# sm-edwards/CrossScale-ECG-A-Modular-HPC-Pipeline-from-Locality-Optimization-to-MPI-GPU-Overlap

Hardware: AMD Instinct MI355X
Metric: ECG samples/sec (node) + conv1d speedup vs torch.Conv1d, tiny 1D-CNN at 1/2/4/8 GPU (higher is better)
Workload: dtype bf16; 1 GPU; model=TinyECG (1458 params), global_batch=256, seq_len=500, parallelism=dp1, sync=fedavg every 50 local steps (none all_reduce AVG, overlap=none), per_client_batch=256, max_windows_per_client=20000, backend=fused

## Files before the change

### crossscale-ecg-a-modular-hpc-pipeline-from-locality-optimization-to-mpi-gpu-overlap_amd/ops/_lib.py

```python
from __future__ import annotations

import ctypes as C
import os
import threading
from typing import Optional

import torch

LIB_DIR = os.environ.get("ECG_LIB_DIR") or os.path.join(os.path.dirname(os.path.dirname(os.path.abspath(__file__))), "_lib")

_lock = threading.Lock()
_libs = {}

vp, i32, i64, f32 = C.c_void_p, C.c_int, C.c_long, C.c_float
u64 = C.c_uint64
f64p = C.POINTER(C.c_double)
i32p = C.POINTER(C.c_int)
i64p = C.POINTER(C.c_int64)

STATUS = {0: "ok", 1: "bad argument", 2: "problem too large for the fused kernel", 3: "HIP runtime error",
          4: "I/O error", 5: "timeout", 6: "end of data"}


class NativeError(RuntimeError):
# ... 9 lines not shown
    with _lock:
        if name in _libs:
            return _libs[name]
        path = os.path.join(LIB_DIR, name)
        lib = None
        if os.path.exists(path):
            lib = C.CDLL(path, mode=C.RTLD_GLOBAL)
        _libs[name] = lib
        return lib


def _sig(lib, name, argtypes, restype=i32):
    fn = getattr(lib, name)
    fn.argtypes = argtypes
    fn.restype = restype
    return fn


class TinyRound(C.Structure):
    _fields_ = [("X", vp), ("ldx", i64), ("idx", vp), ("Y", vp), ("params", vp), ("mom", vp), ("slab", vp),
                ("loss_acc", vp), ("wprep", vp), ("xg", vp), ("yg", vp),
                ("L", i32), ("nc", i32), ("slab_stride", i32), ("B", i32), ("steps", i32),
                ("lr", f32), ("momentum", f32), ("wd", f32), ("nesterov", i32), ("prec", i32),
                ("dp_clip", f32), ("dp_sigma", f32), ("dp_seed", u64), ("dp_scale", vp), ("dp_step", vp)]


def _bind_kernels(lib: C.CDLL) -> None:
    _sig(lib, "ecg_tiny_param_count", [i32])
    _sig(lib, "ecg_tiny_smem_bytes", [i32, i32])
    _sig(lib, "ecg_tiny_step_grads", [vp, i32, i64, vp, vp, vp, i32, vp, i32, i32, f32, i32, vp, vp])
    _sig(lib, "ecg_tiny_forward", [vp, i32, i64, vp, vp, i32, vp, i32, i32, vp, vp])
    _sig(lib, "ecg_tiny_wprep_bytes", [])
    _sig(lib, "ecg_tiny_prep", [vp, vp, vp])
    _sig(lib, "ecg_tiny_eval", [vp, i32, i64, vp, vp, i32, vp, i32, vp, vp, vp, vp, vp, i32, vp])
    _sig(lib, "ecg_tiny_eval_scratch_bytes", [i32])
    _sig(lib, "ecg_tiny_eval_out_bytes", [i32])
    _sig(lib, "ecg_slab_reduce_sgd", [vp, i32, i32, i32, vp, vp, vp, vp, f32, f32, f32, i32, i32, vp, vp])
    _sig(lib, "ecg_slab_reduce_dp_sgd", [vp, i32, i32, i32, vp, vp, vp, vp, f32, f32, f32, i32, i32, vp,
                                         f32, f32, u64, vp, vp, vp])
    _sig(lib, "ecg_dp_noise", [vp, i32, u64, u64, vp])
    native = _sig(lib, "ecg_tiny_round_sizeof", [])()
    if native != C.sizeof(TinyRound):
        raise NativeError(f"EcgTinyRound is {native} bytes in libecg_kernels.so but {C.sizeof(TinyRound)} in "
                          "ops/_lib.py: rebuild the library (python csrc/build.py) or update TinyRound")
    _sig(lib, "ecg_tiny_round_enqueue", [C.POINTER(TinyRound), vp])
    _sig(lib, "ecg_tiny_round_capture", [C.POINTER(vp), C.POINTER(TinyRound)])
    _sig(lib, "ecg_tiny_gather_floats", [i32, i32], i64)
    _sig(lib, "ecg_tiny_step_grads_twice", [vp, i32, i64, vp, vp, vp, i32, vp, i32, i32, f32, i32, vp, vp])
    _sig(lib, "ecg_tiny_force_waves", [i32])
    _sig(lib, "ecg_tiny_set_stamps", [vp])
    _sig(lib, "ecg_round_graph_launch", [vp, vp])
    _sig(lib, "ecg_round_graph_destroy", [vp])
    _sig(lib, "ecg_round_graph_upload", [vp, vp])
    _sig(lib, "conv1d_batch_hip", [vp, vp, vp, i32, i32, i32, vp])
    _sig(lib, "conv1d_batch_hip_sync", [vp, vp, vp, i32, i32, i32, vp])
    _sig(lib, "conv1d_batch_hip_spin", [vp, vp, vp, i32, i32, i32, vp])
    _sig(lib, "conv1d_batch_hip_flag", [vp, vp, vp, i32, i32, i32, vp])
    _sig(lib, "conv1d_valid_dgrad_hip", [vp, vp, vp, i32, i32, i32, vp])
    _sig(lib, "conv1d_valid_dgrad_hip_bf16", [vp, vp, vp, i32, i32, i32, vp])
    _sig(lib, "conv1d_valid_wgrad_ws_floats", [i32, i32, i32], i64)
    _sig(lib, "conv1d_valid_wgrad_hip", [vp, vp, vp, vp, i64, i32, i32, i32, vp])
    _sig(lib, "conv1d_valid_wgrad_hip_bf16", [vp, vp, vp, vp, i64, i32, i32, i32, vp])
    _sig(lib, "conv1d_batch_hip_bf16", [vp, vp, vp, i32, i32, i32, vp])
    _sig(lib, "ecg_sgd_flat", [vp, vp, vp, i64, f32, f32, f32, f32, i32, i32, f32, vp, vp])
    _sig(lib, "ecg_gather_rows_f32", [vp, i64, i32, vp, i32, vp, i64, i32, f32, vp])
    _sig(lib, "ecg_gather_rows_bf16", [vp, i64, i32, vp, i32, vp, i64, i32, f32, vp])
    for extra in ("_bind_conv_mc",):
        fn = globals().get(extra)
        if fn:
            fn(lib)
# ... 91 lines not shown
```

### crossscale-ecg-a-modular-hpc-pipeline-from-locality-optimization-to-mpi-gpu-overlap_amd/ops/fused_tiny.py

```python
from __future__ import annotations

import ctypes as C
import os
from typing import Optional

import torch

from . import _lib
from ..models.tiny_ecg import TinyECG, num_params
from ..data.dataset import DeviceIndexSampler
from ..utils.philox import mix64
from .tiny_eval import EvalResult, TinyEvaluator, evaluate_torch, tiny_evaluate


PRECISION = {"bf16": 0, "fp32": 1}


def prec_id(precision: str) -> int:
    if precision not in PRECISION:
        raise ValueError(f"precision must be one of {list(PRECISION)}, got {precision!r}")
    return PRECISION[precision]


def new_wprep(device) -> torch.Tensor:
# ... 94 lines not shown
    z = torch.empty(P, dtype=torch.float32, device=device)
    st = _lib.kernels().ecg_dp_noise(z.data_ptr(), P, int(seed) & (2 ** 64 - 1), int(t) & (2 ** 64 - 1),
                                     _lib.stream_ptr(z.device))
    _lib.check(st, "ecg_dp_noise")
    return z


def reduce_slab(slab: torch.Tensor, num_classes: int = 2):
    P = num_params(num_classes)
    grad = torch.empty(P, dtype=torch.float32, device=slab.device)
    loss = torch.zeros(1, dtype=torch.float32, device=slab.device)
    lib = _lib.kernels()
    st = lib.ecg_slab_reduce_sgd(slab.data_ptr(), slab.shape[0], slab.shape[1], P, None, None, grad.data_ptr(),
                                 loss.data_ptr(), 0.0, 0.0, 0.0, 0, 0, None, _lib.stream_ptr(slab.device))
    _lib.check(st, "ecg_slab_reduce_sgd")
    return grad, loss


class FusedTinyTrainer:

    def __init__(self, model: TinyECG, x_gpu: torch.Tensor, y_gpu: torch.Tensor, batch_size: int,
                 steps_per_round: int, lr: float = 1e-2, momentum: float = 0.9, weight_decay: float = 0.0,
                 nesterov: bool = False, seed: Optional[int] = None, use_graph: Optional[bool] = None,
                 precision: str = "bf16", prefrag: bool = True, gather: bool = True,
                 dp_clip: float = 0.0, dp_noise: float = 0.0, dp_seed: Optional[int] = None):
        self.device = x_gpu.device
        self.precision = precision
        self.prec = prec_id(precision)
        self.model = model
        self.nc = model.num_classes
        self.params = model.flat if model.flat is not None else model.flatten_parameters()
        if self.params.device != self.device:
            raise ValueError("model and dataset must be on the same device")
        self.P = num_params(self.nc)
        self.x = x_gpu.contiguous()
        self.y32 = labels_int32(y_gpu, self.nc)
        _check_dataset(self.x, self.y32, self.nc)
        self.B = int(batch_size)
        self.S = int(steps_per_round)
        self.lr, self.momentum, self.wd, self.nesterov = float(lr), float(momentum), float(weight_decay), bool(nesterov)
        self.stride = slab_stride(self.nc)
        self.mom = torch.zeros_like(self.params)
        self.slab = torch.empty((self.B, self.stride), dtype=torch.float32, device=self.device)
        self.loss_acc = torch.zeros(1, dtype=torch.float32, device=self.device)
        self.idx_table = torch.zeros((self.S, self.B), dtype=torch.int32, device=self.device)
        self.idx_stage = torch.zeros((self.S, self.B), dtype=torch.int32, device=self.device)
        self._staged: Optional[int] = None
        self._loss_steps = 0
        self.sampler = DeviceIndexSampler(self.x.shape[0], self.B, self.device, seed=seed)
        self.use_graph = (os.environ.get("ECG_TINY_GRAPH", "1") != "0") if use_graph is None else bool(use_graph)
        self._graphs = {}
        self.steps_done = 0
        self._evaluator: Optional[TinyEvaluator] = None
        lib = _lib.kernels()
        L = self.x.shape[1]
        smem = lib.ecg_tiny_smem_bytes(L, self.prec)
        if smem > 160 * 1024:
            raise ValueError(f"window length {L} too long for the fused kernel ({smem} B LDS)")
        self.prefrag = bool(prefrag) and precision == "bf16"
        self.wprep = new_wprep(self.device) if self.prefrag else None
        self.gather = bool(gather) and self.prefrag
        self.xg = self.yg = None
        if self.gather:
            self.xg = torch.zeros(lib.ecg_tiny_gather_floats(L, self.B), dtype=torch.float32, device=self.device)
            self.yg = torch.zeros(2 * self.B, dtype=torch.int32, device=self.device)
        check_dp_args(dp_clip, dp_noise)
        self.dp_clip, self.dp_noise = float(dp_clip), float(dp_noise)
        self.dp = self.dp_clip > 0.0
        self.dp_seed = (mix64(0 if seed is None else seed) if dp_seed is None else int(dp_seed)) & (2 ** 64 - 1)
        self.dp_steps = 0
        self.dp_scale = self.dp_step = None
        if self.dp:
            self.dp_scale = torch.zeros(self.B, dtype=torch.float32, device=self.device)
            self.dp_step = torch.zeros(1, dtype=torch.int64, device=self.device)
        self._round = _lib.TinyRound(
            X=self.x.data_ptr(), ldx=self.x.stride(0), Y=self.y32.data_ptr(), params=self.params.data_ptr(),
            mom=self.mom.data_ptr(), slab=self.slab.data_ptr(), loss_acc=self.loss_acc.data_ptr(),
            wprep=_lib.ptr(self.wprep), xg=_lib.ptr(self.xg), yg=_lib.ptr(self.yg), L=L, nc=self.nc,
            slab_stride=self.stride, B=self.B, lr=self.lr, momentum=self.momentum, wd=self.wd,
            nesterov=int(self.nesterov), prec=self.prec, dp_clip=self.dp_clip, dp_sigma=self.dp_noise,
            dp_seed=self.dp_seed, dp_scale=_lib.ptr(self.dp_scale), dp_step=_lib.ptr(self.dp_step))

    def _round_of(self, n: int, table: torch.Tensor):
        r = self._round
        r.idx, r.steps = table.data_ptr(), n
        return C.byref(r)

    def _graph_for(self, n: int, table: torch.Tensor) -> C.c_void_p:
        key = (n, table.data_ptr())
        g = self._graphs.get(key)
        if g is None:
            g = C.c_void_p()
            torch.cuda.synchronize(self.device)
            _lib.check(_lib.kernels().ecg_tiny_round_capture(C.byref(g), self._round_of(n, table)),
                       "ecg_tiny_round_capture")
            self._graphs[key] = g
        return g

    def close(self):
        graphs, self._graphs = getattr(self, "_graphs", {}), {}
        for g in graphs.values():
            if g.value:
                _lib.kernels().ecg_round_graph_destroy(g)

# ... 100 lines not shown
```

### csrc/kernels/tiny_ecg_step.hip

```cpp
#include "../include/ecg_common.h"
#include "../include/tiny_ecg.h"

#include <climits>
#include <cstdint>
#include <cstdlib>
#include <cstring>
#include <type_traits>

namespace {

using namespace ecg::tiny;

constexpr int MAX_PAIRS_PER_WAVE = 4;

struct Smem {
  int Lp;
  int xs_off, xcol_off, h1_off, dh2_off, ps_off, frag_off, red_off, bytes;
};

constexpr int RED_G = 0;
constexpr int RED_POOLED = 16;
constexpr int RED_POOL = 48;

struct FusedOpt {
  int slab_wt;
};
__host__ __device__ constexpr int msplit(int waves) { return (waves - 1) / 5 < 1 ? 1 : (waves - 1) / 5; }
__host__ __device__ constexpr int red_cnt(int waves) { return RED_POOL + waves * 16; }
__host__ __device__ constexpr int red_m(int waves) { return red_cnt(waves) + waves * 16; }
__host__ __device__ constexpr int red_dw1(int waves) { return red_m(waves) + msplit(waves) * 1280; }
__host__ __device__ constexpr int red_head(int waves) { return red_dw1(waves) + waves * 128; }
__host__ __device__ constexpr int red_floats(int waves) { return red_head(waves) + 288; }

__device__ __forceinline__ void st_wt(__amdgpu_buffer_rsrc_t r, int idx, float v) {
  __builtin_amdgcn_raw_buffer_store_b32(__builtin_bit_cast(unsigned, v), r, idx * 4, 0, 16);
}
__device__ __forceinline__ void st_wt4(__amdgpu_buffer_rsrc_t r, int idx, f32x4 v) {
  typedef int i32x4 __attribute__((ext_vector_type(4)));
  __builtin_amdgcn_raw_buffer_store_b128(__builtin_bit_cast(i32x4, v), r, idx * 4, 0, 16);
}
__device__ __forceinline__ float ld_wt(__amdgpu_buffer_rsrc_t r, int idx) {
  return __builtin_bit_cast(float, __builtin_amdgcn_raw_buffer_load_b32(r, idx * 4, 0, 16));
}
constexpr int kOobByte = 0x40000000;

constexpr int F32_KSTEPS = C * K2 / 4;

__host__ __device__ constexpr bool frag_pad_is_bias(int which, int l, int j) { return which == 0 && j == 0 && l < 48; }

__device__ __forceinline__ void wprep_put(unsigned char* wp, int i, float v) {
  __bf16* wb = reinterpret_cast<__bf16*>(wp);
  if (i < C * K1) {
    wb[WP_AW1 + (i / K1) * 8 + i % K1] = ecg::to_bf16(v);
  } else if (i < C * K1 + C) {
    wb[WP_AW1 + (i - C * K1) * 8 + 7] = ecg::to_bf16(v);
  } else if (i < kParamsW2End) {
    const int e = i - (C * K1 + C);
    const int co = e / (C * K2), ci = (e / K2) % C, k = e % K2;
    const int rf = 16 * k + ci, rd = 16 * k + co;
    const __bf16 bv = ecg::to_bf16(v);
    wb[WP_FRAGF + ((rf >> 5) * 64 + 16 * ((rf & 31) >> 3) + co) * 8 + (rf & 7)] = bv;
    wb[WP_FRAGD + ((rd >> 5) * 64 + 16 * ((rd & 31) >> 3) + ci) * 8 + (rd & 7)] = bv;
  } else if (i < kParamsW2End + C) {
    reinterpret_cast<float*>(wp + WP_B2_BYTE)[i - kParamsW2End] = v;
    wb[WP_FRAGF + frag_bias_elem(i - kParamsW2End)] = ecg::to_bf16(v);
  }
}
// ... 17 lines not shown
  s.h1_off = s.xcol_off + (f32 ? 0 : (s.Lp + 1) * 16);
  const int act_bytes = (s.Lp + 8) * C * (f32 ? 4 : 2);
  s.dh2_off = s.h1_off + act_bytes;
  s.ps_off = s.dh2_off + act_bytes;
  const int ps_bytes = ((make_layout(nc).P) * 4 + 15) / 16 * 16;
  s.frag_off = s.ps_off + ps_bytes;
  s.red_off = s.frag_off + (f32 ? 2 * F32_KSTEPS * 64 * 4 : 2 * 3 * 64 * 16);
  s.bytes = s.red_off + (red_floats(waves) * 4 + 15) / 16 * 16;
  return s;
}

__device__ __forceinline__ bf16x8 cat44(s16x4 a, s16x4 b) {
  typedef short s16x8 __attribute__((ext_vector_type(8)));
  s16x8 r;
  r[0] = a[0]; r[1] = a[1]; r[2] = a[2]; r[3] = a[3];
  r[4] = b[0]; r[5] = b[1]; r[6] = b[2]; r[7] = b[3];
  return __builtin_bit_cast(bf16x8, r);
}

__device__ __forceinline__ s16x4 lds_tr16(const __bf16* p) {
  return __builtin_amdgcn_ds_read_tr16_b64_v4i16((__attribute__((address_space(3))) s16x4*)(p));
}

template <int WAVES, bool F32, bool PF = false>
struct TinySample {
  static_assert(!(PF && F32), "prepared fragments are bf16 operands");
  using AT = std::conditional_t<F32, float, __bf16>;
  static constexpr int NT = WAVES * 64;
  Smem sm;
  Layout lay;
  int L, Lp, NP, nc;
  int tid, lane, w, h, c;
  float* xs;
  __bf16* xcol;
  AT* h1s;
  AT* ms;
  float* ps;
  __bf16* fragF;
  __bf16* fragD;
  float* fragF32;
  float* fragD32;
  float* red;
  uint32_t mask1 = 0u;
  bf16x8 pf_aw, pf_wf[3], pf_wd[3];

  __device__ __forceinline__ void load_aw(const float* __restrict__ params) {
#pragma unroll
    for (int j = 0; j < 8; ++j) {
      const float v = j < K1 ? params[lay.w1 + c * K1 + j] : params[lay.b1 + c];
// ... 48 lines not shown
  __device__ __forceinline__ void load_x(const float* __restrict__ xrow, XRegs& r) const {
#pragma unroll
    for (int k = 0; k < XK; ++k) {
      const int i = tid + k * NT, t = i - 3;
      if (k * NT < Lp + 16) {
        const float v = xrow[min(max(t, 0), L - 1)];
        r.v[k] = (i < Lp + 16 && t >= 0 && t < L) ? v : 0.f;
      }
    }
  }
  __device__ __forceinline__ void put_x(const XRegs& r) {
#pragma unroll
    for (int k = 0; k < XK; ++k) {
      const int i = tid + k * NT;
      if (i < Lp + 16) xs[i] = r.v[k];
    }
  }
  __device__ __forceinline__ void stage_x(const float* __restrict__ xrow) {
    XRegs r;
    load_x(xrow, r);
    put_x(r);
  }

  struct X1 {
    float v[2][K1];
  };
  __device__ __forceinline__ int conv1_t(int pi, int u) const {
    return 16 * min(w + (pi + u) * WAVES, Lp / 16 - 1) + (lane & 15);
  }
  __device__ __forceinline__ void conv1_load(__amdgpu_buffer_rsrc_t xr, int pi, X1& r) const {
#pragma unroll
    for (int u = 0; u < 2; ++u) {
      const int t = conv1_t(pi, u);
      const int base = (h == 0 && t < L) ? 4 * max(t - 3, 0) : kOobByte;
#pragma unroll
      for (int j = 0; j < K1; ++j) r.v[u][j] = ld_bounded(xr, base + 4 * j);
    }
  }
  __device__ __forceinline__ bf16x8 conv1_operand(const float (&ld)[K1], int t) const {
    float v[K1];
#pragma unroll
    for (int j = 0; j < K1; ++j) v[j] = ld[j];
    if (h == 0 && t < 3) {
      const int s = 3 - t;
#pragma unroll
      for (int j = K1 - 1; j >= 0; --j) v[j] = (s & 1) ? (j >= 1 ? v[j - 1] : 0.f) : v[j];
#pragma unroll
      for (int j = K1 - 1; j >= 0; --j) v[j] = (s & 2) ? (j >= 2 ? v[j - 2] : 0.f) : v[j];
    }
    bf16x8 Bx;
#pragma unroll
    for (int j = 0; j < K1; ++j) Bx[j] = ecg::to_bf16(v[j]);
    Bx[7] = ecg::to_bf16(h == 0 && t < L ? 1.f : 0.f);
    return Bx;
  }

  __device__ __forceinline__ void put_param(int i, float v) {
    ps[i] = v;
    if constexpr (!F32) {
      if (i >= lay.b2 && i < lay.b2 + C) fragF[frag_bias_elem(i - lay.b2)] = ecg::to_bf16(v);
// ... 20 lines not shown
        if (!frag_pad_is_bias(which, l, j)) (which ? fragD : fragF)[(2 * 64 + l) * 8 + j] = ecg::to_bf16(0.f);
      }
      if (tid < 4) reinterpret_cast<uint32_t*>(xcol + Lp * 8)[tid] = 0u;
    }
    constexpr int DW = C * (int)sizeof(AT) / 4;
    uint32_t* h1w = reinterpret_cast<uint32_t*>(h1s);
    uint32_t* mw = reinterpret_cast<uint32_t*>(ms);
    for (int i = tid; i < 8 * DW; i += NT) {
      const int r = i / DW, d = i % DW;
      const int hr = r < 2 ? r : Lp + 2 + (r - 2);
      h1w[hr * DW + d] = 0u;
      const int dr = r < 4 ? r : Lp + 4 + (r - 4);
      mw[dr * DW + d] = 0u;
    }
  }

  __device__ __forceinline__ void conv1_pair(int pi, const X1& x) {
    const bool has2 = w + (pi + 1) * WAVES < Lp / 16;
    bf16x8 Bx[2];
    int t[2];
#pragma unroll
    for (int u = 0; u < 2; ++u) {
      t[u] = conv1_t(pi, u);
      Bx[u] = conv1_operand(x.v[u], t[u]);
      if (h == 0) *reinterpret_cast<bf16x8*>(xcol + t[u] * 8) = Bx[u];
    }
#pragma unroll
    for (int u = 0; u < 2; ++u) {
      if (u == 1 && !has2) break;
      const f32x4 acc = __builtin_amdgcn_mfma_f32_16x16x32_bf16(pf_aw, Bx[u], f32x4{0.f, 0.f, 0.f, 0.f}, 0, 0, 0);
      bf16x4 o;
#pragma unroll
      for (int i = 0; i < 4; ++i) o[i] = (AT)fmaxf(acc[i], 0.f);
      *reinterpret_cast<bf16x4*>(h1s + (t[u] + 2) * C + 4 * h) = o;
    }
  }
  __device__ __forceinline__ void conv1_mfma(__amdgpu_buffer_rsrc_t xr, const X1& x0) {
    const int ntiles = Lp / 16;
    if (w < ntiles) conv1_pair(0, x0);
#pragma unroll 1
    for (int pi = 2; pi < 2 * MAX_PAIRS_PER_WAVE; pi += 2) {
      if (w + pi * WAVES >= ntiles) break;
      X1 x;
      conv1_load(xr, pi, x);
      conv1_pair(pi, x);
    }
  }
// ... 412 lines not shown

  __device__ __forceinline__ void row_store(__amdgpu_buffer_rsrc_t r, int rowbase) const {
    constexpr int NQ = C * C * K2 / 4;
    static_assert(NQ + 128 + C <= NT || WAVES < 16, "one job per thread at 16 waves");
    if (tid < NQ) {
      const int e0 = 4 * tid;
      f32x4 v = *reinterpret_cast<const f32x4*>(red + red_m(WAVES) + e0);
#pragma unroll
      for (int part = 1; part < msplit(WAVES); ++part) {
        const f32x4 u = *reinterpret_cast<const f32x4*>(red + red_m(WAVES) + part * 1280 + e0);
        v[0] += u[0]; v[1] += u[1]; v[2] += u[2]; v[3] += u[3];
      }
      const float g = red[RED_G + e0 / (C * K2)];
#pragma unroll
      for (int q = 0; q < 4; ++q) v[q] *= g;
      st_wt4(r, rowbase + lay.w2 + e0, v);
    } else {
      const int i = tid < NQ + 128 ? tid - NQ : lay.b2 + (tid - NQ - 128);
      if (i <= lay.P) st_wt(r, rowbase + i, row_value(i));
    }
  }
};

template <int WAVES, int MODE, bool F32, bool PF>
__global__ __launch_bounds__(WAVES * 64) void tiny_ecg_step_kernel(
    const float* __restrict__ X, int L, long ldx,
    const int* __restrict__ idx,
    const int* __restrict__ Y,
    const float* __restrict__ params, int nc,
    float* __restrict__ out, int out_stride,
    float inv_B, unsigned long long* __restrict__ stamps,
    FusedOpt opt, const unsigned char* __restrict__ wprep) {
  extern __shared__ __attribute__((aligned(16))) unsigned char smem[];
  TinySample<WAVES, F32, PF> S(smem, L, nc);
  constexpr bool TRAIN = MODE != 1;
  const int tid = threadIdx.x;
  const int b = blockIdx.x;
  const __amdgpu_buffer_rsrc_t slab_r = make_rsrc(out, (long)gridDim.x * out_stride * 4);
  const int rowbase = b * out_stride;
  if (stamps && tid == 0) stamps[(long)b * 16 + 15] = __builtin_amdgcn_s_memrealtime();
#pragma unroll 1
  for (int rep = 0; rep < (MODE == 2 ? 2 : 1); ++rep) {
#define ECG_STAMP(k) \
  if (stamps && tid == 0) stamps[(long)b * 16 + 7 * rep + (k)] = __builtin_amdgcn_s_memtime();
    ECG_STAMP(0)
    int ylab = 0;
    const long row = idx ? (long)idx[b] : (long)b;
    const float* xrow = X + row * ldx;
    [[maybe_unused]] const __amdgpu_buffer_rsrc_t xr = make_rsrc(xrow, (long)L * 4);
    [[maybe_unused]] typename TinySample<WAVES, F32, PF>::X1 x0;
    if constexpr (PF) {
      S.pf_load_fwd(wprep);
      const int i = S.lay.wh + tid;
      const float hv = i < S.lay.P ? params[i] : 0.f;
      if (TRAIN) ylab = Y[row];
      S.conv1_load(xr, 0, x0);
      if (i < S.lay.P) S.ps[i] = hv;
      static_assert(MAX_CLASSES * C + MAX_CLASSES <= 8 * 64, "head parameters: one per thread");
    } else {
      constexpr int PR = 4;
      float pv[PR];
#pragma unroll
      for (int j = 0; j < PR; ++j) {
        const int i = tid + j * S.NT;
        pv[j] = i < S.lay.P ? params[i] : 0.f;
      }
      if constexpr (!F32) S.load_aw(params);
      if (TRAIN) ylab = Y[row];
      if constexpr (F32) {
        S.stage_x(xrow);
      } else {
        S.conv1_load(xr, 0, x0);
      }
// ... 34 lines not shown
      for (int i = tid; i <= S.lay.P; i += S.NT) st_wt(slab_r, rowbase + i, S.row_value(i));
    } else {
      for (int i = tid; i <= S.lay.P; i += S.NT) out[rowbase + i] = S.row_value(i);
    }
    ECG_STAMP(6)
#undef ECG_STAMP
    if (MODE == 2) __syncthreads();
  }
  if (stamps && tid == 0) stamps[(long)b * 16 + 14] = __builtin_amdgcn_s_memrealtime();
}

constexpr int kRedColsDefault = 32;
constexpr int RED_ROWG = 16;

struct GatherArgs {
  const float* X;
  long ldx;
  const int* idx;
  const int* Y;
  float* xg;
  int* yg;
  int L, ldg, B, vec;
  int nred;
};
__host__ __device__ inline int gather_rows_per_block(int L, int vec, int nt) {
  const int per_row = vec ? L / 4 : L;
  return per_row >= nt ? 1 : nt / per_row;
}

template <int RED_COLS>
__global__ __launch_bounds__(RED_COLS * RED_ROWG) void slab_reduce_sgd_kernel(
    const float* __restrict__ slab, int G, int stride, int P,
    float* __restrict__ params, float* __restrict__ mom, float* __restrict__ grad_out,
    float* __restrict__ loss_acc, float lr, float momentum, float wd, int nesterov, int apply,
    unsigned char* __restrict__ wprep,
    GatherArgs ga) {
  constexpr int NT = RED_COLS * RED_ROWG;
  if ((int)blockIdx.x >= ga.nred) {
    const int per_row = ga.vec ? ga.L / 4 : ga.L;
    const int rpb = gather_rows_per_block(ga.L, ga.vec, NT);
    const int r0 = ((int)blockIdx.x - ga.nred) * rpb;
    const __amdgpu_buffer_rsrc_t xr = make_rsrc(ga.xg, (long)ga.B * ga.ldg * 4);
    for (int e = threadIdx.x; e < rpb * per_row; e += NT) {
      const int lr_ = e / per_row, j = e - lr_ * per_row, b = r0 + lr_;
      if (b >= ga.B) break;
      const long row = ga.idx[b];
      if (ga.vec) {
        st_wt4(xr, b * ga.ldg + 4 * j, *reinterpret_cast<const f32x4*>(ga.X + row * ga.ldx + 4 * j));
      } else {
        st_wt(xr, b * ga.ldg + j, ga.X[row * ga.ldx + j]);
      }
      if (j == 0) ga.yg[b] = ga.Y[row];
    }
    return;
  }
  __shared__ float part[RED_ROWG][RED_COLS + 1];
  const int cl = threadIdx.x % RED_COLS, rg = threadIdx.x / RED_COLS;
  const int col = blockIdx.x * RED_COLS + cl;
  const bool upd = rg == 0 && col < P && apply;
  const float p0 = upd ? params[col] : 0.f;
  const float m0 = (upd && momentum != 0.f) ? mom[col] : 0.f;
  float s = 0.f;
  if (col <= P) {
    const float* base = slab + col;
    int r = rg;
    for (; r + RED_ROWG * 15 < G; r += RED_ROWG * 16) {
      float v[16];
#pragma unroll
      for (int j = 0; j < 16; ++j) v[j] = base[(long)(r + RED_ROWG * j) * stride];
#pragma unroll
      for (int j = 0; j < 16; j += 2) s += v[j] + v[j + 1];
    }
    for (; r < G; r += RED_ROWG) s += base[(long)r * stride];
  }
  part[rg][cl] = s;
  __syncthreads();
// ... 69 lines not shown
  } else {
    for (int c0 = lane; c0 < P; c0 += 64) {
      const float v = row[c0];
      ss += v * v;
    }
  }
#pragma unroll
  for (int o = 32; o > 0; o >>= 1) ss += __shfl_xor(ss, o, 64);
  if (lane == 0) {
    const float n = (float)G * sqrtf(ss);
    scale[b] = n > 0.f ? fminf(1.f, clip / n) : 1.f;
  }
}

template <int RED_COLS>
__global__ __launch_bounds__(RED_COLS * RED_ROWG) void slab_reduce_dp_sgd_kernel(
    const float* __restrict__ slab, int G, int stride, int P,
    float* __restrict__ params, float* __restrict__ mom, float* __restrict__ grad_out,
    float* __restrict__ loss_acc, float lr, float momentum, float wd, int nesterov, int apply,
    unsigned char* __restrict__ wprep, const float* __restrict__ scale, float noise_scale, unsigned long long seed,
    const unsigned long long* __restrict__ dp_step, GatherArgs ga) {
  constexpr int NT = RED_COLS * RED_ROWG;
  if ((int)blockIdx.x >= ga.nred) {
    const int per_row = ga.vec ? ga.L / 4 : ga.L;
    const int rpb = gather_rows_per_block(ga.L, ga.vec, NT);
    const int r0 = ((int)blockIdx.x - ga.nred) * rpb;
    const __amdgpu_buffer_rsrc_t xr = make_rsrc(ga.xg, (long)ga.B * ga.ldg * 4);
    for (int e = threadIdx.x; e < rpb * per_row; e += NT) {
      const int lr_ = e / per_row, j = e - lr_ * per_row, b = r0 + lr_;
      if (b >= ga.B) break;
      const long row = ga.idx[b];
      if (ga.vec) {
        st_wt4(xr, b * ga.ldg + 4 * j, *reinterpret_cast<const f32x4*>(ga.X + row * ga.ldx + 4 * j));
      } else {
        st_wt(xr, b * ga.ldg + j, ga.X[row * ga.ldx + j]);
      }
      if (j == 0) ga.yg[b] = ga.Y[row];
    }
    return;
  }
  __shared__ float part[RED_ROWG][RED_COLS + 1];
  const int cl = threadIdx.x % RED_COLS, rg = threadIdx.x / RED_COLS;
  const int col = blockIdx.x * RED_COLS + cl;
  const bool upd = rg == 0 && col < P && apply;
  const float p0 = upd ? params[col] : 0.f;
  const float m0 = (upd && momentum != 0.f) ? mom[col] : 0.f;
  float noise = 0.f;
  if (rg == 0 && col < P && noise_scale != 0.f) noise = noise_scale * dp_normal(col, seed, dp_step[0] - 1ull);
  float s = 0.f;
  if (col <= P) {
    const float* base = slab + col;
    const bool grad_col = col < P;
    int r = rg;
    for (; r + RED_ROWG * 15 < G; r += RED_ROWG * 16) {
      float v[16];
#pragma unroll
      for (int j = 0; j < 16; ++j) {
        const int rr = r + RED_ROWG * j;
        v[j] = base[(long)rr * stride] * (grad_col ? scale[rr] : 1.f);
      }
#pragma unroll
// ... 28 lines not shown
  }
}

unsigned long long* g_stamps = nullptr;

FusedOpt no_fuse() {
  FusedOpt o{};
  o.slab_wt = 1;
  return o;
}

struct StepArgs {
  const float* X;
  int L;
  long ldx;
  const int* idx;
  const int* Y;
  const float* params;
  int nc;
  float* out;
  int out_stride, B;
  float inv_B;
  const unsigned char* wprep;
};

template <int WAVES, int MODE, bool F32, bool PF>
int launch_step(const StepArgs& a, hipStream_t stream) {
  const Smem sm = make_smem(a.L, WAVES, a.nc, F32);
  auto kern = tiny_ecg_step_kernel<WAVES, MODE, F32, PF>;
  if (sm.bytes > 64 * 1024)
    ECG_HIP_CHECK(hipFuncSetAttribute((const void*)kern, hipFuncAttributeMaxDynamicSharedMemorySize, sm.bytes));
  hipLaunchKernelGGL(kern, dim3(a.B), dim3(WAVES * 64), sm.bytes, stream, a.X, a.L, a.ldx, a.idx, a.Y, a.params, a.nc,
                     a.out, a.out_stride, a.inv_B, g_stamps, no_fuse(), PF ? a.wprep : nullptr);
  ECG_HIP_CHECK(hipGetLastError());
  return ecg::kOk;
}

int launch_prep(const float* params, unsigned char* wprep, hipStream_t stream) {
  if (!params || !wprep) return ecg::kBadArg;
  hipLaunchKernelGGL(tiny_prep_kernel, dim3(1), dim3(256), 0, stream, params, wprep);
  ECG_HIP_CHECK(hipGetLastError());
  return ecg::kOk;
}

constexpr int kMaxLds = 160 * 1024;

int g_forced_waves = 0;
int pick_waves(int L, bool f32) {
  const int Lp = (L + 31) / 32 * 32;
  const int forced = g_forced_waves;
  const bool fit16 = Lp <= 32 * 4 * 16 && make_smem(L, 16, MAX_CLASSES, f32).bytes <= kMaxLds;
  if (forced == 16 && fit16) return 16;
// ... 5 lines not shown
  if (L < 8 || B <= 0 || nc < 1 || nc > MAX_CLASSES) return ecg::kBadArg;
  const int Lp = (L + 31) / 32 * 32;
  if (Lp > 32 * 4 * 8 || make_smem(L, 8, MAX_CLASSES, f32).bytes > kMaxLds) return ecg::kTooLarge;
  const Layout lay = make_layout(nc);
  if (mode != 1 && out_stride < lay.P + 1) return ecg::kBadArg;
  if (mode == 1 && out_stride < nc) return ecg::kBadArg;
  return ecg::kOk;
}

template <bool F32, bool PF>
int dispatch_cfg(int mode, int waves, const StepArgs& a, hipStream_t stream) {
  if (mode == 2)
    return launch_step<8, 2, F32, PF>(a, stream);
  if (mode == 0) return waves == 8 ? launch_step<8, 0, F32, PF>(a, stream) : launch_step<16, 0, F32, PF>(a, stream);
  return waves == 8 ? launch_step<8, 1, F32, PF>(a, stream) : launch_step<16, 1, F32, PF>(a, stream);
}

int step_dispatch(int mode, int prec, const StepArgs& a, hipStream_t stream) {
  if (prec != 0 && prec != 1) return ecg::kBadArg;
  int st = check_step_args(a.L, a.nc, a.B, a.out_stride, mode, prec == 1);
  if (st) return st;
  if (a.wprep && prec == 1) return ecg::kBadArg;
  const int waves = pick_waves(a.L, prec == 1);
  if (prec == 1) return dispatch_cfg<true, false>(mode, waves, a, stream);
  if (a.wprep) return dispatch_cfg<false, true>(mode, waves, a, stream);
  return dispatch_cfg<false, false>(mode, waves, a, stream);
}

int reduce_dispatch(const float* slab, int G, int stride, int P, float* params, float* mom, float* grad_out,
                    float* loss_acc, float lr, float momentum, float wd, int nesterov, int apply,
                    unsigned char* wprep, hipStream_t stream, const GatherArgs* gather = nullptr) {
  if (G <= 0 || P <= 0 || stride < P + 1) return ecg::kBadArg;
  if (apply && (!params || (momentum != 0.f && !mom))) return ecg::kBadArg;
  constexpr int cols = kRedColsDefault;
  const int blocks = (P + 1 + cols - 1) / cols;
  GatherArgs ga{};
  ga.nred = INT_MAX;
  int grid = blocks;
  if (gather) {
    ga = *gather;
    ga.nred = blocks;
    const int rpb = gather_rows_per_block(ga.L, ga.vec, cols * RED_ROWG);
    grid += (ga.B + rpb - 1) / rpb;
  }
  hipLaunchKernelGGL(slab_reduce_sgd_kernel<cols>, dim3(grid), dim3(cols * RED_ROWG), 0, stream, slab, G, stride, P,
                     params, mom, grad_out, loss_acc, lr, momentum, wd, nesterov, apply, wprep, ga);
// ... 125 lines not shown
  ECG_HIP_CHECK(hipGetLastError());
  return ecg::kOk;
}

struct EcgTinyRound {
  const float* X;
  long ldx;
  const int* idx;
  const int* Y;
  float* params;
  float* mom;
  float* slab;
  float* loss_acc;
  void* wprep;
  float* xg;
  int* yg;
  int L, nc, slab_stride, B, steps;
  float lr, momentum, wd;
  int nesterov, prec;
  float dp_clip, dp_sigma;
  unsigned long long dp_seed;
  float* dp_scale;
  unsigned long long* dp_step;
};

ECG_API int ecg_tiny_round_sizeof(void) { return (int)sizeof(EcgTinyRound); }

static int check_round(const EcgTinyRound* r) {
  if (!r || r->steps < 1 || !r->X || !r->Y || !r->params || !r->slab) return ecg::kBadArg;
  if (r->prec != 0 && r->prec != 1) return ecg::kBadArg;
  if (r->wprep && r->prec != 0) return ecg::kBadArg;
  if ((!r->xg) != (!r->yg) || (r->xg && (!r->wprep || !r->idx))) return ecg::kBadArg;
  if (r->dp_clip < 0.f || r->dp_sigma < 0.f || (r->dp_sigma > 0.f && r->dp_clip == 0.f)) return ecg::kBadArg;
  if (r->dp_clip > 0.f && (!r->dp_scale || !r->dp_step)) return ecg::kBadArg;
  return check_step_args(r->L, r->nc, r->B, r->slab_stride, 0, r->prec == 1);
}

static int enqueue_round(const EcgTinyRound& r, hipStream_t stream) {
  const int P = make_layout(r.nc).P;
  unsigned char* wprep = static_cast<unsigned char*>(r.wprep);
  const int ldg = (r.L + 3) / 4 * 4;
  GatherArgs ga{r.X, r.ldx, nullptr, r.Y, nullptr, nullptr, r.L, ldg, r.B,
                (r.L % 4 == 0 && r.ldx % 4 == 0 && reinterpret_cast<uintptr_t>(r.X) % 16 == 0) ? 1 : 0, INT_MAX};
  for (int s = 0; s < r.steps; ++s) {
    const int* idx = r.idx ? r.idx + (long)s * r.B : nullptr;
    const bool gathered = r.xg && s > 0;
    const bool gather_next = r.xg && s + 1 < r.steps;
    if (gather_next) {
      ga.idx = idx + r.B;
      ga.xg = r.xg + (long)((s + 1) & 1) * r.B * ldg;
      ga.yg = r.yg + (long)((s + 1) & 1) * r.B;
    }
    StepArgs a{r.X, r.L, r.ldx, idx, r.Y, r.params, r.nc, r.slab, r.slab_stride, r.B, 1.0f / (float)r.B,
               s == 0 ? nullptr : wprep};
    if (gathered) {
      a.X = r.xg + (long)(s & 1) * r.B * ldg;
      a.ldx = ldg;
      a.idx = nullptr;
      a.Y = r.yg + (long)(s & 1) * r.B;
    }
    int st = step_dispatch(0, r.prec, a, stream);
    if (st) return st;
    if (r.dp_clip > 0.f)
      st = dp_reduce_dispatch(r.slab, r.B, r.slab_stride, P, r.params, r.mom, nullptr, r.loss_acc, r.lr, r.momentum,
                              r.wd, r.nesterov, 1, wprep, {r.dp_clip, r.dp_sigma, r.dp_seed, r.dp_scale, r.dp_step},
                              stream, gather_next ? &ga : nullptr);
    else
      st = reduce_dispatch(r.slab, r.B, r.slab_stride, P, r.params, r.mom, nullptr, r.loss_acc, r.lr, r.momentum, r.wd,
                           r.nesterov, 1, wprep, stream, gather_next ? &ga : nullptr);
    if (st) return st;
  }
  return ecg::kOk;
}

ECG_API int ecg_tiny_round_enqueue(const EcgTinyRound* round, hipStream_t stream) {
  const int st = check_round(round);
  return st ? st : enqueue_round(*round, stream);
}

ECG_API int ecg_tiny_round_capture(void** handle, const EcgTinyRound* round) {
  if (!handle) return ecg::kBadArg;
  int st = check_round(round);
// ... 8 lines not shown
    (void)hipStreamDestroy(cap);
    return ecg::kHipError;
  }
  st = enqueue_round(*round, cap);
  e = hipStreamEndCapture(cap, &rg->graph);
  (void)hipStreamDestroy(cap);
  if (st != 0 || e != hipSuccess) {
    if (rg->graph) (void)hipGraphDestroy(rg->graph);
    delete rg;
    return st ? st : ecg::kHipError;
  }
  e = hipGraphInstantiate(&rg->exec, rg->graph, nullptr, nullptr, 0);
  if (e != hipSuccess) {
    (void)hipGraphDestroy(rg->graph);
    delete rg;
    return ecg::kHipError;
  }
  *handle = rg;
  return ecg::kOk;
}

ECG_API long ecg_tiny_gather_floats(int L, int B) { return 2L * B * ((L + 3) / 4 * 4); }

ECG_API int ecg_round_graph_launch(void* handle, hipStream_t stream) {
  if (!handle) return ecg::kBadArg;
  RoundGraph* rg = static_cast<RoundGraph*>(handle);
  ECG_HIP_CHECK(hipGraphLaunch(rg->exec, stream));
  return ecg::kOk;
}

ECG_API int ecg_round_graph_upload(void* handle, hipStream_t stream) {
  if (!handle) return ecg::kBadArg;
  RoundGraph* rg = static_cast<RoundGraph*>(handle);
  ECG_HIP_CHECK(hipGraphUpload(rg->exec, stream));
  return ecg::kOk;
}

ECG_API int ecg_round_graph_destroy(void* handle) {
  if (!handle) return ecg::kOk;
  RoundGraph* rg = static_cast<RoundGraph*>(handle);
  if (rg->exec) (void)hipGraphExecDestroy(rg->exec);
  if (rg->graph) (void)hipGraphDestroy(rg->graph);
  delete rg;
  return ecg::kOk;
}
```

Measured before the change: 25.32 million samples/s.

## Pack gathered windows as padded bf16 rows for the prepared-fragment step kernel

The gather blocks in the reduce kernel now also write each gathered window as a zero-padded bf16 row with a 4-element lead. The next step kernel reads its conv1 operands from that row with one 128-bit load per tile and builds them with alignbit/perm, replacing seven bounded fp32 loads and converts. This halves the input bytes the step reads and drops the per-element conversion, at the cost of extra bf16 stores in the gather and a second staging buffer.

```diff
diff --git a/crossscale-ecg-a-modular-hpc-pipeline-from-locality-optimization-to-mpi-gpu-overlap_amd/ops/_lib.py b/crossscale-ecg-a-modular-hpc-pipeline-from-locality-optimization-to-mpi-gpu-overlap_amd/ops/_lib.py
--- a/crossscale-ecg-a-modular-hpc-pipeline-from-locality-optimization-to-mpi-gpu-overlap_amd/ops/_lib.py
+++ b/crossscale-ecg-a-modular-hpc-pipeline-from-locality-optimization-to-mpi-gpu-overlap_amd/ops/_lib.py
@@ -55,7 +55,8 @@
                 ("loss_acc", vp), ("wprep", vp), ("xg", vp), ("yg", vp),
                 ("L", i32), ("nc", i32), ("slab_stride", i32), ("B", i32), ("steps", i32),
                 ("lr", f32), ("momentum", f32), ("wd", f32), ("nesterov", i32), ("prec", i32),
-                ("dp_clip", f32), ("dp_sigma", f32), ("dp_seed", u64), ("dp_scale", vp), ("dp_step", vp)]
+                ("dp_clip", f32), ("dp_sigma", f32), ("dp_seed", u64), ("dp_scale", vp), ("dp_step", vp),
+                ("xbg", vp)]
 
 
 def _bind_kernels(lib: C.CDLL) -> None:
@@ -79,6 +80,7 @@
     _sig(lib, "ecg_tiny_round_enqueue", [C.POINTER(TinyRound), vp])
     _sig(lib, "ecg_tiny_round_capture", [C.POINTER(vp), C.POINTER(TinyRound)])
     _sig(lib, "ecg_tiny_gather_floats", [i32, i32], i64)
+    _sig(lib, "ecg_tiny_gather_halfs", [i32, i32], i64)
     _sig(lib, "ecg_tiny_step_grads_twice", [vp, i32, i64, vp, vp, vp, i32, vp, i32, i32, f32, i32, vp, vp])
     _sig(lib, "ecg_tiny_force_waves", [i32])
     _sig(lib, "ecg_tiny_set_stamps", [vp])
diff --git a/crossscale-ecg-a-modular-hpc-pipeline-from-locality-optimization-to-mpi-gpu-overlap_amd/ops/fused_tiny.py b/crossscale-ecg-a-modular-hpc-pipeline-from-locality-optimization-to-mpi-gpu-overlap_amd/ops/fused_tiny.py
--- a/crossscale-ecg-a-modular-hpc-pipeline-from-locality-optimization-to-mpi-gpu-overlap_amd/ops/fused_tiny.py
+++ b/crossscale-ecg-a-modular-hpc-pipeline-from-locality-optimization-to-mpi-gpu-overlap_amd/ops/fused_tiny.py
@@ -140,7 +140,7 @@
     def __init__(self, model: TinyECG, x_gpu: torch.Tensor, y_gpu: torch.Tensor, batch_size: int,
                  steps_per_round: int, lr: float = 1e-2, momentum: float = 0.9, weight_decay: float = 0.0,
                  nesterov: bool = False, seed: Optional[int] = None, use_graph: Optional[bool] = None,
-                 precision: str = "bf16", prefrag: bool = True, gather: bool = True,
+                 precision: str = "bf16", prefrag: bool = True, gather: bool = True, pack: bool = True,
                  dp_clip: float = 0.0, dp_noise: float = 0.0, dp_seed: Optional[int] = None):
         self.device = x_gpu.device
         self.precision = precision
@@ -182,6 +182,10 @@
         if self.gather:
             self.xg = torch.zeros(lib.ecg_tiny_gather_floats(L, self.B), dtype=torch.float32, device=self.device)
             self.yg = torch.zeros(2 * self.B, dtype=torch.int32, device=self.device)
+        self.pack = bool(pack) and self.gather
+        self.xbg = None
+        if self.pack:
+            self.xbg = torch.zeros(lib.ecg_tiny_gather_halfs(L, self.B), dtype=torch.bfloat16, device=self.device)
         check_dp_args(dp_clip, dp_noise)
         self.dp_clip, self.dp_noise = float(dp_clip), float(dp_noise)
         self.dp = self.dp_clip > 0.0
@@ -197,7 +201,8 @@
             wprep=_lib.ptr(self.wprep), xg=_lib.ptr(self.xg), yg=_lib.ptr(self.yg), L=L, nc=self.nc,
             slab_stride=self.stride, B=self.B, lr=self.lr, momentum=self.momentum, wd=self.wd,
             nesterov=int(self.nesterov), prec=self.prec, dp_clip=self.dp_clip, dp_sigma=self.dp_noise,
-            dp_seed=self.dp_seed, dp_scale=_lib.ptr(self.dp_scale), dp_step=_lib.ptr(self.dp_step))
+            dp_seed=self.dp_seed, dp_scale=_lib.ptr(self.dp_scale), dp_step=_lib.ptr(self.dp_step),
+            xbg=_lib.ptr(self.xbg))
 
     def _round_of(self, n: int, table: torch.Tensor):
         r = self._round
diff --git a/csrc/kernels/tiny_ecg_step.hip b/csrc/kernels/tiny_ecg_step.hip
--- a/csrc/kernels/tiny_ecg_step.hip
+++ b/csrc/kernels/tiny_ecg_step.hip
@@ -32,6 +32,9 @@
 __host__ __device__ constexpr int red_head(int waves) { return red_dw1(waves) + waves * 128; }
 __host__ __device__ constexpr int red_floats(int waves) { return red_head(waves) + 288; }
 
+typedef unsigned u32x4 __attribute__((ext_vector_type(4)));
+typedef unsigned u32x2 __attribute__((ext_vector_type(2)));
+
 __device__ __forceinline__ void st_wt(__amdgpu_buffer_rsrc_t r, int idx, float v) {
   __builtin_amdgcn_raw_buffer_store_b32(__builtin_bit_cast(unsigned, v), r, idx * 4, 0, 16);
 }
@@ -39,10 +42,19 @@
   typedef int i32x4 __attribute__((ext_vector_type(4)));
   __builtin_amdgcn_raw_buffer_store_b128(__builtin_bit_cast(i32x4, v), r, idx * 4, 0, 16);
 }
+__device__ __forceinline__ void st_wt_b64(__amdgpu_buffer_rsrc_t r, int byte_off, u32x2 v) {
+  __builtin_amdgcn_raw_buffer_store_b64(v, r, byte_off, 0, 16);
+}
+__device__ __forceinline__ void st_wt_b16(__amdgpu_buffer_rsrc_t r, int byte_off, unsigned short v) {
+  __builtin_amdgcn_raw_buffer_store_b16(v, r, byte_off, 0, 16);
+}
 __device__ __forceinline__ float ld_wt(__amdgpu_buffer_rsrc_t r, int idx) {
   return __builtin_bit_cast(float, __builtin_amdgcn_raw_buffer_load_b32(r, idx * 4, 0, 16));
 }
 constexpr int kOobByte = 0x40000000;
+
+constexpr int kPackLead = 4;
+__host__ __device__ constexpr int pack_ldb(int L) { return (L + 31) / 32 * 32 + 8; }
 
 constexpr int F32_KSTEPS = C * K2 / 4;
 
@@ -106,9 +118,10 @@
   return __builtin_amdgcn_ds_read_tr16_b64_v4i16((__attribute__((address_space(3))) s16x4*)(p));
 }
 
-template <int WAVES, bool F32, bool PF = false>
+template <int WAVES, bool F32, bool PF = false, bool PK = false>
 struct TinySample {
   static_assert(!(PF && F32), "prepared fragments are bf16 operands");
+  static_assert(!PK || PF, "packed window rows feed the prepared-fragment kernel only");
   using AT = std::conditional_t<F32, float, __bf16>;
   static constexpr int NT = WAVES * 64;
   Smem sm;
@@ -203,20 +216,44 @@
     put_x(r);
   }
 
-  struct X1 {
+  struct X1f {
     float v[2][K1];
   };
+  struct X1p {
+    u32x4 p[2];
+  };
+  using X1 = std::conditional_t<PK, X1p, X1f>;
   __device__ __forceinline__ int conv1_t(int pi, int u) const {
     return 16 * min(w + (pi + u) * WAVES, Lp / 16 - 1) + (lane & 15);
   }
   __device__ __forceinline__ void conv1_load(__amdgpu_buffer_rsrc_t xr, int pi, X1& r) const {
-#pragma unroll
-    for (int u = 0; u < 2; ++u) {
-      const int t = conv1_t(pi, u);
-      const int base = (h == 0 && t < L) ? 4 * max(t - 3, 0) : kOobByte;
-#pragma unroll
-      for (int j = 0; j < K1; ++j) r.v[u][j] = ld_bounded(xr, base + 4 * j);
-    }
+    if constexpr (PK) {
+#pragma unroll
+      for (int u = 0; u < 2; ++u) {
+        const int t = conv1_t(pi, u);
+        const int off = (h == 0 && t < L) ? 2 * ((t + kPackLead - 3) & ~1) : kOobByte;
+        r.p[u] = __builtin_bit_cast(u32x4, __builtin_amdgcn_raw_buffer_load_b128(xr, off, 0, 0));
+      }
+    } else {
+#pragma unroll
+      for (int u = 0; u < 2; ++u) {
+        const int t = conv1_t(pi, u);
+        const int base = (h == 0 && t < L) ? 4 * max(t - 3, 0) : kOobByte;
+#pragma unroll
+        for (int j = 0; j < K1; ++j) r.v[u][j] = ld_bounded(xr, base + 4 * j);
+      }
+    }
+  }
+  __device__ __forceinline__ bf16x8 conv1_operand_packed(u32x4 d, int t) const {
+    static_assert(kPackLead % 2 == 0, "the shift below assumes an even lead: window start t + kPackLead - 3");
+    const bool odd = !(lane & 1);
+    const unsigned sh = odd ? 16u : 0u;
+    const unsigned flag = (h == 0 && t < L) ? 0x3f80u : 0u;
+    u32x4 o;
+#pragma unroll
+    for (int i = 0; i < 3; ++i) o[i] = __builtin_amdgcn_alignbit(d[i + 1], d[i], sh);
+    o[3] = __builtin_amdgcn_perm(flag, d[3], odd ? 0x05040302u : 0x05040100u);
+    return __builtin_bit_cast(bf16x8, o);
   }
   __device__ __forceinline__ bf16x8 conv1_operand(const float (&ld)[K1], int t) const {
     float v[K1];
@@ -283,7 +320,10 @@
 #pragma unroll
     for (int u = 0; u < 2; ++u) {
       t[u] = conv1_t(pi, u);
-      Bx[u] = conv1_operand(x.v[u], t[u]);
+      if constexpr (PK)
+        Bx[u] = conv1_operand_packed(x.p[u], t[u]);
+      else
+        Bx[u] = conv1_operand(x.v[u], t[u]);
       if (h == 0) *reinterpret_cast<bf16x8*>(xcol + t[u] * 8) = Bx[u];
     }
 #pragma unroll
@@ -742,7 +782,7 @@
   }
 };
 
-template <int WAVES, int MODE, bool F32, bool PF>
+template <int WAVES, int MODE, bool F32, bool PF, bool PK = false>
 __global__ __launch_bounds__(WAVES * 64) void tiny_ecg_step_kernel(
     const float* __restrict__ X, int L, long ldx,
     const int* __restrict__ idx,
@@ -752,7 +792,7 @@
     float inv_B, unsigned long long* __restrict__ stamps,
     FusedOpt opt, const unsigned char* __restrict__ wprep) {
   extern __shared__ __attribute__((aligned(16))) unsigned char smem[];
-  TinySample<WAVES, F32, PF> S(smem, L, nc);
+  TinySample<WAVES, F32, PF, PK> S(smem, L, nc);
   constexpr bool TRAIN = MODE != 1;
   const int tid = threadIdx.x;
   const int b = blockIdx.x;
@@ -767,8 +807,8 @@
     int ylab = 0;
     const long row = idx ? (long)idx[b] : (long)b;
     const float* xrow = X + row * ldx;
-    [[maybe_unused]] const __amdgpu_buffer_rsrc_t xr = make_rsrc(xrow, (long)L * 4);
-    [[maybe_unused]] typename TinySample<WAVES, F32, PF>::X1 x0;
+    [[maybe_unused]] const __amdgpu_buffer_rsrc_t xr = make_rsrc(xrow, PK ? ldx * 4 : (long)L * 4);
+    [[maybe_unused]] typename TinySample<WAVES, F32, PF, PK>::X1 x0;
     if constexpr (PF) {
       S.pf_load_fwd(wprep);
       const int i = S.lay.wh + tid;
@@ -849,11 +889,50 @@
   int* yg;
   int L, ldg, B, vec;
   int nred;
+  __bf16* xbg;
+  int ldb;
 };
 __host__ __device__ inline int gather_rows_per_block(int L, int vec, int nt) {
   const int per_row = vec ? L / 4 : L;
   return per_row >= nt ? 1 : nt / per_row;
 }
+
+template <int NT>
+__device__ __forceinline__ void gather_block(const GatherArgs& ga) {
+  const int per_row = ga.vec ? ga.L / 4 : ga.L;
+  const int rpb = gather_rows_per_block(ga.L, ga.vec, NT);
+  const int r0 = ((int)blockIdx.x - ga.nred) * rpb;
+  const __amdgpu_buffer_rsrc_t xr = make_rsrc(ga.xg, (long)ga.B * ga.ldg * 4);
+  const __amdgpu_buffer_rsrc_t br = make_rsrc(ga.xbg, ga.xbg ? (long)ga.B * ga.ldb * 2 : 0);
+  const int npad = ga.ldb - ga.L;
+  for (int e = threadIdx.x; e < rpb * per_row; e += NT) {
+    const int lr_ = e / per_row, j = e - lr_ * per_row, b = r0 + lr_;
+    if (b >= ga.B) break;
+    const long row = ga.idx[b];
+    if (ga.vec) {
+      const f32x4 v = *reinterpret_cast<const f32x4*>(ga.X + row * ga.ldx + 4 * j);
+      st_wt4(xr, b * ga.ldg + 4 * j, v);
+      if (ga.xbg) {
+        bf16x4 p;
+#pragma unroll
+        for (int q = 0; q < 4; ++q) p[q] = ecg::to_bf16(v[q]);
+        st_wt_b64(br, (b * ga.ldb + kPackLead + 4 * j) * 2, __builtin_bit_cast(u32x2, p));
+        for (int u = j; u < npad / 4; u += per_row)
+          st_wt_b64(br, (b * ga.ldb + (u == 0 ? 0 : ga.L + 4 * u)) * 2, u32x2{0u, 0u});
+      }
+    } else {
+      const float v = ga.X[row * ga.ldx + j];
+      st_wt(xr, b * ga.ldg + j, v);
+      if (ga.xbg) {
+        st_wt_b16(br, (b * ga.ldb + kPackLead + j) * 2, __builtin_bit_cast(unsigned short, ecg::to_bf16(v)));
+        for (int u = j; u < npad; u += per_row)
+          st_wt_b16(br, (b * ga.ldb + (u < kPackLead ? u : ga.L + u)) * 2, (unsigned short)0);
+      }
+    }
+    if (j == 0) ga.yg[b] = ga.Y[row];
+  }
+}
+static_assert(kPackLead == 4, "gather_block's 4-float form writes the lead as one 8-byte unit");
 
 template <int RED_COLS>
 __global__ __launch_bounds__(RED_COLS * RED_ROWG) void slab_reduce_sgd_kernel(
@@ -864,21 +943,7 @@
     GatherArgs ga) {
   constexpr int NT = RED_COLS * RED_ROWG;
   if ((int)blockIdx.x >= ga.nred) {
-    const int per_row = ga.vec ? ga.L / 4 : ga.L;
-    const int rpb = gather_rows_per_block(ga.L, ga.vec, NT);
-    const int r0 = ((int)blockIdx.x - ga.nred) * rpb;
-    const __amdgpu_buffer_rsrc_t xr = make_rsrc(ga.xg, (long)ga.B * ga.ldg * 4);
-    for (int e = threadIdx.x; e < rpb * per_row; e += NT) {
-      const int lr_ = e / per_row, j = e - lr_ * per_row, b = r0 + lr_;
-      if (b >= ga.B) break;
-      const long row = ga.idx[b];
-      if (ga.vec) {
-        st_wt4(xr, b * ga.ldg + 4 * j, *reinterpret_cast<const f32x4*>(ga.X + row * ga.ldx + 4 * j));
-      } else {
-        st_wt(xr, b * ga.ldg + j, ga.X[row * ga.ldx + j]);
-      }
-      if (j == 0) ga.yg[b] = ga.Y[row];
-    }
+    gather_block<NT>(ga);
     return;
   }
   __shared__ float part[RED_ROWG][RED_COLS + 1];
@@ -994,21 +1059,7 @@
     const unsigned long long* __restrict__ dp_step, GatherArgs ga) {
   constexpr int NT = RED_COLS * RED_ROWG;
   if ((int)blockIdx.x >= ga.nred) {
-    const int per_row = ga.vec ? ga.L / 4 : ga.L;
-    const int rpb = gather_rows_per_block(ga.L, ga.vec, NT);
-    const int r0 = ((int)blockIdx.x - ga.nred) * rpb;
-    const __amdgpu_buffer_rsrc_t xr = make_rsrc(ga.xg, (long)ga.B * ga.ldg * 4);
-    for (int e = threadIdx.x; e < rpb * per_row; e += NT) {
-      const int lr_ = e / per_row, j = e - lr_ * per_row, b = r0 + lr_;
-      if (b >= ga.B) break;
-      const long row = ga.idx[b];
-      if (ga.vec) {
-        st_wt4(xr, b * ga.ldg + 4 * j, *reinterpret_cast<const f32x4*>(ga.X + row * ga.ldx + 4 * j));
-      } else {
-        st_wt(xr, b * ga.ldg + j, ga.X[row * ga.ldx + j]);
-      }
-      if (j == 0) ga.yg[b] = ga.Y[row];
-    }
+    gather_block<NT>(ga);
     return;
   }
   __shared__ float part[RED_ROWG][RED_COLS + 1];
@@ -1083,12 +1134,13 @@
   int out_stride, B;
   float inv_B;
   const unsigned char* wprep;
+  bool packed = false;
 };
 
-template <int WAVES, int MODE, bool F32, bool PF>
+template <int WAVES, int MODE, bool F32, bool PF, bool PK = false>
 int launch_step(const StepArgs& a, hipStream_t stream) {
   const Smem sm = make_smem(a.L, WAVES, a.nc, F32);
-  auto kern = tiny_ecg_step_kernel<WAVES, MODE, F32, PF>;
+  auto kern = tiny_ecg_step_kernel<WAVES, MODE, F32, PF, PK>;
   if (sm.bytes > 64 * 1024)
     ECG_HIP_CHECK(hipFuncSetAttribute((const void*)kern, hipFuncAttributeMaxDynamicSharedMemorySize, sm.bytes));
   hipLaunchKernelGGL(kern, dim3(a.B), dim3(WAVES * 64), sm.bytes, stream, a.X, a.L, a.ldx, a.idx, a.Y, a.params, a.nc,
@@ -1140,6 +1192,11 @@
   if (st) return st;
   if (a.wprep && prec == 1) return ecg::kBadArg;
   const int waves = pick_waves(a.L, prec == 1);
+  if (a.packed) {
+    if (mode != 0 || prec != 0 || !a.wprep || a.idx) return ecg::kBadArg;
+    return waves == 8 ? launch_step<8, 0, false, true, true>(a, stream)
+                      : launch_step<16, 0, false, true, true>(a, stream);
+  }
   if (prec == 1) return dispatch_cfg<true, false>(mode, waves, a, stream);
   if (a.wprep) return dispatch_cfg<false, true>(mode, waves, a, stream);
   return dispatch_cfg<false, false>(mode, waves, a, stream);
@@ -1311,6 +1368,7 @@
   unsigned long long dp_seed;
   float* dp_scale;
   unsigned long long* dp_step;
+  void* xbg;
 };
 
 ECG_API int ecg_tiny_round_sizeof(void) { return (int)sizeof(EcgTinyRound); }
@@ -1320,6 +1378,7 @@
   if (r->prec != 0 && r->prec != 1) return ecg::kBadArg;
   if (r->wprep && r->prec != 0) return ecg::kBadArg;
   if ((!r->xg) != (!r->yg) || (r->xg && (!r->wprep || !r->idx))) return ecg::kBadArg;
+  if (r->xbg && !r->xg) return ecg::kBadArg;
   if (r->dp_clip < 0.f || r->dp_sigma < 0.f || (r->dp_sigma > 0.f && r->dp_clip == 0.f)) return ecg::kBadArg;
   if (r->dp_clip > 0.f && (!r->dp_scale || !r->dp_step)) return ecg::kBadArg;
   return check_step_args(r->L, r->nc, r->B, r->slab_stride, 0, r->prec == 1);
@@ -1329,8 +1388,11 @@
   const int P = make_layout(r.nc).P;
   unsigned char* wprep = static_cast<unsigned char*>(r.wprep);
   const int ldg = (r.L + 3) / 4 * 4;
+  const int ldb = pack_ldb(r.L);
+  __bf16* xbg = static_cast<__bf16*>(r.xbg);
   GatherArgs ga{r.X, r.ldx, nullptr, r.Y, nullptr, nullptr, r.L, ldg, r.B,
-                (r.L % 4 == 0 && r.ldx % 4 == 0 && reinterpret_cast<uintptr_t>(r.X) % 16 == 0) ? 1 : 0, INT_MAX};
+                (r.L % 4 == 0 && r.ldx % 4 == 0 && reinterpret_cast<uintptr_t>(r.X) % 16 == 0) ? 1 : 0, INT_MAX,
+                nullptr, ldb};
   for (int s = 0; s < r.steps; ++s) {
     const int* idx = r.idx ? r.idx + (long)s * r.B : nullptr;
     const bool gathered = r.xg && s > 0;
@@ -1339,6 +1401,7 @@
       ga.idx = idx + r.B;
       ga.xg = r.xg + (long)((s + 1) & 1) * r.B * ldg;
       ga.yg = r.yg + (long)((s + 1) & 1) * r.B;
+      ga.xbg = xbg ? xbg + (long)((s + 1) & 1) * r.B * ldb : nullptr;
     }
     StepArgs a{r.X, r.L, r.ldx, idx, r.Y, r.params, r.nc, r.slab, r.slab_stride, r.B, 1.0f / (float)r.B,
                s == 0 ? nullptr : wprep};
@@ -1347,6 +1410,11 @@
       a.ldx = ldg;
       a.idx = nullptr;
       a.Y = r.yg + (long)(s & 1) * r.B;
+      if (xbg) {
+        a.X = reinterpret_cast<const float*>(xbg + (long)(s & 1) * r.B * ldb);
+        a.ldx = ldb / 2;
+        a.packed = true;
+      }
     }
     int st = step_dispatch(0, r.prec, a, stream);
     if (st) return st;
@@ -1401,6 +1469,8 @@
 
 ECG_API long ecg_tiny_gather_floats(int L, int B) { return 2L * B * ((L + 3) / 4 * 4); }
 
+ECG_API long ecg_tiny_gather_halfs(int L, int B) { return 2L * B * pack_ldb(L); }
+
 ECG_API int ecg_round_graph_launch(void* handle, hipStream_t stream) {
   if (!handle) return ecg::kBadArg;
   RoundGraph* rg = static_cast<RoundGraph*>(handle);
```

Measured after the change: 25.62 million samples/s (median of 6 runs). +1.2%, better.
